# pratyushkumar211/industrial_nnmpc_2021

Measured on AMD Instinct MI355X. Metric: condensed-QP solves/sec (CDU offline datagen), higher is better.
Workload: dtype f64; 1 GPU; cdu_offline_data: synthetic CDU-size plant (n=4480 vars, m=8960 box rows, n_aug=284), 100000 sampled x0 per GPU per step, whole sequences u* written out; batch_per_gpu=100000, total_batch=100000, method=auto, parallelism=dp1 (sharded samples, 1 RCCL gather of the first moves pe...

## Files before the change

industrial_nnmpc_2021_amd/csrc/qp_asm.h:

```cpp
#pragma once
#include <hip/hip_runtime.h>
#include <stdint.h>
#include <type_traits>

#if defined(ASM_WG_TU) && ASM_WG_TU >= 0
#define ASM_OWN_KERNELS 0
#else
#define ASM_OWN_KERNELS 1
#endif

namespace nnmpc {

constexpr int ASM_MLDS = 176;
constexpr int ASM_TS = 16 * 17;
enum { ASM_RUN = 0, ASM_DONE = 1, ASM_FALLBACK = 2, ASM_CERT = 3, ASM_WIDE = 4, ASM_INVALID = 5 };
constexpr int ASM_NBIN = 8;
constexpr int ASM_NREG = 6;
constexpr int ASM_NCNT = 40;
constexpr int ASM_CNT_F32 = 16;
constexpr int ASM_NLIST = 2 * ASM_NBIN;
constexpr int ASM_BIG32 = 256;
constexpr int ASM_CNT_BIG64 = 37;
constexpr int ASM_CNT_BIG32 = 36;
constexpr int ASM_BIG32B = 384;
// ... 376 lines not shown
  if (tid == 0) *s_bad = 0;
  const size_t o = (size_t)p * d.np;
  const unsigned char* st = d.st + (size_t)p * d.n;
  const int mb = (m + 15) / 16;
  __syncthreads();
  for (int i = tid; i < mb * 16; i += 256) {
    double v = 0.0;
    if (i < m) {
      const int a = idx[i], k = a % d.nu;
      v = d.xunc[o + a] - (st[a] == 1 ? d.ub[(size_t)p * d.nu + k] : d.lb[(size_t)p * d.nu + k]);
    }
    rA[i] = v;
  }
  const int ntile = mb * (mb + 1) / 2;
  {
    const int ti = tid >> 4, tj = tid & 15;
    int I = 0, J = 0;
    for (int t0 = 0; t0 < ntile; t0 += 4) {
      double v[4];
      int tI[4], tJ[4];
#pragma unroll
      for (int u = 0; u < 4; ++u) {
        tI[u] = I; tJ[u] = J;
        const int gi = 16 * I + ti, gj = 16 * J + tj;
        v[u] = gi == gj ? 1.0 : 0.0;
        if (t0 + u < ntile && gi < m && gj < m) v[u] = d.H[(size_t)idx[gi] * d.np + idx[gj]];
        if (++J > I) { J = 0; ++I; }
      }
#pragma unroll
      for (int u = 0; u < 4; ++u)
        if (t0 + u < ntile) asm_tile(T, tI[u], tJ[u])[ti * 17 + tj] = v[u];
    }
  }
  __syncthreads();
  for (int K = 0; K < mb; ++K) {
    double* TKK = asm_tile(T, K, K);
    if (wave == 0) {
      const int bad = asm_diag16_call(TKK, Yt, lane);
      if (bad && lane == 0) *s_bad = 1;
    }
    __syncthreads();
    for (int I = K + 1 + wave; I < mb; I += 4) {
      double* TIK = asm_tile(T, I, K);
      const f64x4_t acc = tile_mma_nt(TIK, Yt, lane);
#pragma unroll
      for (int r = 0; r < 4; ++r) TIK[((lane >> 4) + 4 * r) * 17 + (lane & 15)] = acc[r];
    }
    __syncthreads();
    {
      int b = 0;
      for (int I = K + 1; I < mb; ++I)
        for (int J = K + 1; J <= I; ++J, ++b) {
          if ((b & 3) != wave) continue;
          const f64x4_t acc = tile_mma_nt(asm_tile(T, I, K), asm_tile(T, J, K), lane);
          double* TIJ = asm_tile(T, I, J);
#pragma unroll
          for (int r = 0; r < 4; ++r) TIJ[((lane >> 4) + 4 * r) * 17 + (lane & 15)] -= acc[r];
        }
    }
    if (wave == 0 && lane < 16) {
      const int row = lane;
#pragma unroll
      for (int k = 0; k < 16; ++k) if (k >= row) TKK[row * 17 + k] = Yt[k * 17 + row];
    }
    __syncthreads();
  }
  if (*s_bad) return 1;
  if (wave == 0) {
    const int i = lane & 15, kq = lane >> 4;
    for (int K = 0; K < mb; ++K) {
      double t = 0.0;
      for (int J = 0; J < K; ++J) {
        const double* TKJ = asm_tile(T, K, J);
#pragma unroll
        for (int k = 0; k < 4; ++k) t += TKJ[i * 17 + 4 * kq + k] * rA[16 * J + 4 * kq + k];
      }
      t += __shfl_xor(t, 16); t += __shfl_xor(t, 32);
      t = rA[16 * K + i] - t;
      const double* TKK = asm_tile(T, K, K);
      double yv = t * TKK[i * 17 + i];
#pragma unroll
      for (int k = 0; k < 16; ++k) { const double tk = __shfl(t, k); if (k < i) yv += TKK[k * 17 + i] * tk; }
      if (lane < 16) rA[16 * K + i] = yv;
      asm volatile("s_waitcnt lgkmcnt(0)" ::: "memory");
    }
    for (int K = mb - 1; K >= 0; --K) {
      double t = 0.0;
      for (int I = K + 1; I < mb; ++I) {
        const double* TIK = asm_tile(T, I, K);
#pragma unroll
        for (int k = 0; k < 4; ++k) t += TIK[(4 * kq + k) * 17 + i] * rA[16 * I + 4 * kq + k];
      }
      t += __shfl_xor(t, 16); t += __shfl_xor(t, 32);
      t = rA[16 * K + i] - t;
      const double* TKK = asm_tile(T, K, K);
      double lv = t * TKK[i * 17 + i];
#pragma unroll
      for (int k = 0; k < 16; ++k) { const double tk = __shfl(t, k); if (k > i) lv += TKK[i * 17 + k] * tk; }
      if (lane < 16) rA[16 * K + i] = lv;
      asm volatile("s_waitcnt lgkmcnt(0)" ::: "memory");
    }
  }
  __syncthreads();
  return 0;
}

#if ASM_OWN_KERNELS
template <int BIG>
__global__ __launch_bounds__(256, 4) void asm_lambda_tile_k(AsmDev d, int bin) {
  extern __shared__ __attribute__((aligned(16))) double sm[];
  __shared__ int s_bad;
  const int tid = threadIdx.x;
  const int cap = BIG ? d.max_active : asm_bin_cap(bin);
  double* rA = sm;
  double* Yt = rA + cap;
  double* T = BIG ? d.scratch + (size_t)blockIdx.x * ((size_t)(cap / 16) * (cap / 16 + 1) / 2 * ASM_TS)
                  : Yt + ASM_TS;
  const int nitem = BIG ? d.counters[1] : d.counters[4 + bin];
  const int* list = BIG ? d.biglist : d.binlist + (size_t)bin * d.nseg;
  for (int it = blockIdx.x; it < nitem; it += gridDim.x) {
    const int p = list[it];
    const int* idx = d.idxg + (size_t)p * d.max_active;
    const int m = d.mg[p];
    if (asm_tile_solve(d, p, m, idx, rA, Yt, T, &s_bad)) { if (tid == 0) d.state[p] = ASM_FALLBACK; continue; }
    if (tid == 0) d.prec[p] = 1;
    double* lrow = d.lam + (size_t)d.row[p] * d.np;
    for (int i = tid; i < m; i += 256) lrow[idx[i]] = rA[i];
  }
}
#endif

template <class T> struct AsmNum;
typedef float f32x4_t __attribute__((ext_vector_type(4)));
template <> struct AsmNum<double> {
  using v4 = f64x4_t;
  static constexpr bool F32 = false;
  __host__ __device__ static constexpr int kr(int lq, int r) { return lq + 4 * r; }
  __device__ static __forceinline__ v4 mfma(double a, double b, v4 c) { return __builtin_amdgcn_mfma_f64_16x16x4f64(a, b, c, 0, 0, 0); }
  __device__ static __forceinline__ double rdlane(double x, int l) { return rdlane_d(x, l); }
  __device__ static __forceinline__ double rsq(double x) { return rsqrt(x); }

  template <int CTRL> __device__ static __forceinline__ double dpp(double x) {
    const int lo = __builtin_amdgcn_mov_dpp(__double2loint(x), CTRL, 0xf, 0xf, false);
    const int hi = __builtin_amdgcn_mov_dpp(__double2hiint(x), CTRL, 0xf, 0xf, false);
    return __hiloint2double(hi, lo);
  }
  __device__ static __forceinline__ double swap16(double x) {
    const auto a = __builtin_amdgcn_permlane16_swap(__double2loint(x), __double2loint(x), false, false);
    const auto b = __builtin_amdgcn_permlane16_swap(__double2hiint(x), __double2hiint(x), false, false);
    return __hiloint2double(b[0], a[0]) + __hiloint2double(b[1], a[1]);
  }
  __device__ static __forceinline__ double swap32(double x) {
    const auto a = __builtin_amdgcn_permlane32_swap(__double2loint(x), __double2loint(x), false, false);
    const auto b = __builtin_amdgcn_permlane32_swap(__double2hiint(x), __double2hiint(x), false, false);
    return __hiloint2double(b[0], a[0]) + __hiloint2double(b[1], a[1]);
  }
};
template <> struct AsmNum<float> {
  using v4 = f32x4_t;
  static constexpr bool F32 = true;
  __host__ __device__ static constexpr int kr(int lq, int r) { return 4 * lq + r; }
  __device__ static __forceinline__ v4 mfma(float a, float b, v4 c) { return __builtin_amdgcn_mfma_f32_16x16x4f32(a, b, c, 0, 0, 0); }
  __device__ static __forceinline__ float rdlane(float x, int l) { return __int_as_float(__builtin_amdgcn_readlane(__float_as_int(x), l)); }
  __device__ static __forceinline__ float rsq(float x) { return __builtin_amdgcn_rsqf(x); }

  template <int CTRL> __device__ static __forceinline__ float dpp(float x) {
    return __int_as_float(__builtin_amdgcn_mov_dpp(__float_as_int(x), CTRL, 0xf, 0xf, false));
  }
  __device__ static __forceinline__ float swap16(float x) {
    const auto a = __builtin_amdgcn_permlane16_swap(__float_as_int(x), __float_as_int(x), false, false);
    return __int_as_float(a[0]) + __int_as_float(a[1]);
  }
  __device__ static __forceinline__ float swap32(float x) {
    const auto a = __builtin_amdgcn_permlane32_swap(__float_as_int(x), __float_as_int(x), false, false);
    return __int_as_float(a[0]) + __int_as_float(a[1]);
  }
};
template <class T> __device__ __forceinline__ T rowsum16(T x) {
  using N = AsmNum<T>;
  x += N::template dpp<0xB1>(x);
  x += N::template dpp<0x4E>(x);
  x += N::template dpp<0x141>(x);
  x += N::template dpp<0x140>(x);
  return x;
}
template <class T> __device__ __forceinline__ void rowsum16x4(T (&v)[4]) {
#pragma unroll
  for (int r = 0; r < 4; ++r) v[r] = rowsum16<T>(v[r]);
}
template <> __device__ __forceinline__ void rowsum16x4<float>(float (&v)[4]) {
  asm volatile(
      "s_nop 1\n"
      "v_add_f32_dpp %0, %0, %0 quad_perm:[1,0,3,2] row_mask:0xf bank_mask:0xf\n"
      "v_add_f32_dpp %1, %1, %1 quad_perm:[1,0,3,2] row_mask:0xf bank_mask:0xf\n"
      "v_add_f32_dpp %2, %2, %2 quad_perm:[1,0,3,2] row_mask:0xf bank_mask:0xf\n"
      "v_add_f32_dpp %3, %3, %3 quad_perm:[1,0,3,2] row_mask:0xf bank_mask:0xf\n"
      "v_add_f32_dpp %0, %0, %0 quad_perm:[2,3,0,1] row_mask:0xf bank_mask:0xf\n"
      "v_add_f32_dpp %1, %1, %1 quad_perm:[2,3,0,1] row_mask:0xf bank_mask:0xf\n"
      "v_add_f32_dpp %2, %2, %2 quad_perm:[2,3,0,1] row_mask:0xf bank_mask:0xf\n"
      "v_add_f32_dpp %3, %3, %3 quad_perm:[2,3,0,1] row_mask:0xf bank_mask:0xf\n"
      "v_add_f32_dpp %0, %0, %0 row_half_mirror row_mask:0xf bank_mask:0xf\n"
      "v_add_f32_dpp %1, %1, %1 row_half_mirror row_mask:0xf bank_mask:0xf\n"
      "v_add_f32_dpp %2, %2, %2 row_half_mirror row_mask:0xf bank_mask:0xf\n"
      "v_add_f32_dpp %3, %3, %3 row_half_mirror row_mask:0xf bank_mask:0xf\n"
      "v_add_f32_dpp %0, %0, %0 row_mirror row_mask:0xf bank_mask:0xf\n"
      "v_add_f32_dpp %1, %1, %1 row_mirror row_mask:0xf bank_mask:0xf\n"
      "v_add_f32_dpp %2, %2, %2 row_mirror row_mask:0xf bank_mask:0xf\n"
      "v_add_f32_dpp %3, %3, %3 row_mirror row_mask:0xf bank_mask:0xf\n"
      "s_nop 1\n"
      : "+v"(v[0]), "+v"(v[1]), "+v"(v[2]), "+v"(v[3]));
}
template <class T> __device__ __forceinline__ T xsum4(T x) { return AsmNum<T>::swap32(AsmNum<T>::swap16(x)); }

#ifndef ASM_NL_OF_8
#define ASM_NL_OF_8 2
#endif
template <class T> __host__ __device__ constexpr int asm_nl(int mb) {
  return mb <= 7 ? 0 : (mb == 8 ? ASM_NL_OF_8 : (mb <= 9 ? 2 : 4));
}
template <class T> __host__ __device__ constexpr int asm_nlt(int mb) { return asm_nl<T>(mb) * (mb - 1) - asm_nl<T>(mb) * (asm_nl<T>(mb) - 1) / 2; }
template <class T> __host__ __device__ constexpr int asm_rw(int mb) { return 2 * ASM_TS + 2 * mb * 16 + asm_nlt<T>(mb) * 256; }

__host__ __device__ constexpr int asm_tix(int I, int J) { return I * (I + 1) / 2 + J; }
__host__ __device__ constexpr int asm_tri_row(int n, int t) { int J = 0; while (t >= n - J) { t -= n - J; ++J; } return J; }
__host__ __device__ constexpr int asm_tri_col(int n, int t) { int J = 0; while (t >= n - J) { t -= n - J; ++J; } return J + t; }
template <int V> struct asm_ic { static constexpr int value = V; };
template <int B, int E, class F>
__device__ __forceinline__ void asm_sfor(F&& f) {
  if constexpr (B < E) { f(asm_ic<B>{}); asm_sfor<B + 1, E>(f); }
}

template <class T> __device__ __forceinline__ void asm_diag16_begin(T (&x)[16], const T* Tk, const T* Id, int lane) {
  const T* src = lane >= 32 ? Id : Tk;
  const int row = lane & 15;
#pragma unroll
  for (int k = 0; k < 16; ++k) x[k] = src[row * 17 + k];
}
template <class T, int CC> __device__ __forceinline__ void asm_diag16_step(T (&x)[16]) {
  using N = AsmNum<T>;
  const T dd = N::rdlane(x[CC], CC);
  const T w = x[CC] * N::rsq(dd);
  x[CC] = w;
#pragma unroll
  for (int c2 = CC + 1; c2 < 16; ++c2) x[c2] -= w * N::rdlane(w, c2);
}
template <class T> __device__ __forceinline__ int asm_diag16_end(const T (&x)[16], T* Yt, int lane) {
  using N = AsmNum<T>;
  const int bad = !(N::rdlane(x[15], 15) > T(0));
  if (lane >= 48) {
    const int row = lane & 15;
#pragma unroll
    for (int k = 0; k < 16; ++k) Yt[k * 17 + row] = x[k];
  }
  return bad;
}

template <class T>
__device__ __forceinline__ int asm_diag16(const T* Tk, T* Yt, int lane, const T* Id) {
  using N = AsmNum<T>;
  const int row = lane & 15;
  const bool inv_half = lane >= 32;
  T x[16];
  if (Id) {
    const T* src = inv_half ? Id : Tk;
#pragma unroll
    for (int k = 0; k < 16; ++k) x[k] = src[row * 17 + k];
  } else {
#pragma unroll
    for (int k = 0; k < 16; ++k) {
      T a = Tk[row * 17 + k];
      asm volatile("" : "+v"(a));
      x[k] = inv_half ? (k == row ? T(1) : T(0)) : a;
    }
  }
#pragma unroll
  for (int cc = 0; cc < 16; ++cc) {
    const T dd = N::rdlane(x[cc], cc);
    const T w = x[cc] * N::rsq(dd);
    x[cc] = w;
#pragma unroll
    for (int c2 = cc + 1; c2 < 16; ++c2) x[c2] -= w * N::rdlane(w, c2);
  }
  const int bad = !(N::rdlane(x[15], 15) > T(0));
  if (lane >= 48) {
#pragma unroll
    for (int k = 0; k < 16; ++k) Yt[k * 17 + row] = x[k];
  }
  return bad;
}

__device__ __noinline__ int asm_diag16_call(const double* Tk, double* Yt, int lane) { return asm_diag16<double>(Tk, Yt, lane); }


#ifdef ASM_STAMPS
__device__ unsigned long long asm_stamp_buf[64];
#ifndef ASM_STAMP_WG
#define ASM_STAMP_WG 0
#endif
#define ASM_STAMP(i) do { if (wg == ASM_STAMP_WG && wave == 0) { const unsigned long long t_ = __builtin_amdgcn_s_memtime(); if (lane == 0) asm_stamp_buf[i] = t_; } } while (0)
#else
#define ASM_STAMP(i) do { } while (0)
#endif

template <int MB> struct AsmRefine {
  const double *xunc, *lb, *ub;
  const unsigned char* st;
  const int* idx;
  double lam64[MB];
};
template <class T, int MB, int NL, bool ANYM, bool REF>
__device__ __forceinline__ int asm_reg_core(const AsmDev& d, int m, const int* ix, T* dt, T* Yt, T* ys, const T* rv, T* lt, const T* idt,
                                            T (&lam)[MB], int lane, int wg, int wave, AsmRefine<MB>& rf, bool do_refine) {
  using N = AsmNum<T>;
  using V4 = typename N::v4;
  const int li = lane & 15, lq = lane >> 4;
  auto slot = [](int I, int J) { return J * (MB - 1) - J * (J - 1) / 2 + I - J - 1; };
  (void)wg; (void)wave;
  ASM_STAMP(60);
  V4 C[MB * (MB + 1) / 2];
  {
    int gcol[MB];
#pragma unroll
    for (int I = 0; I < MB; ++I) gcol[I] = ix[16 * I + li];
    using HT0 = typename std::conditional<N::F32, float, double>::type;
    const char* const Hbase = N::F32 ? reinterpret_cast<const char*>(d.H32) : reinterpret_cast<const char*>(d.H);
    unsigned gco[MB];
#pragma unroll
    for (int I = 0; I < MB; ++I) gco[I] = (unsigned)gcol[I] * (unsigned)sizeof(HT0);
#pragma unroll
    for (int J = 0; J < MB; ++J) {
#pragma unroll
      for (int r = 0; r < 4; ++r) {
        const int gj = 16 * J + N::kr(lq, r);
        using HT = typename std::conditional<N::F32, float, double>::type;
        const unsigned rowoff = (unsigned)ix[gj] * (unsigned)d.np * (unsigned)sizeof(HT);
#pragma unroll
        for (int I = J; I < MB; ++I) {
          const int gi = 16 * I + li;
          const HT v = *reinterpret_cast<const HT*>(Hbase + (rowoff + gco[I]));
          const bool edge = ANYM || MB <= 4 || I == MB - 1;
          const T e = !edge ? (T)(-v) : ((gi < m && gj < m) ? (T)(-v) : (gi == gj ? T(-1) : T(0)));
          if (J < NL && I > J) lt[slot(I, J) * 256 + r * 64] = e;
          else C[asm_tix(I, J)][r] = e;
        }
      }
      __builtin_amdgcn_sched_barrier(0);
    }
  }
  ASM_STAMP(1);
  T ps[MB];
#pragma unroll
  for (int I = 0; I < MB; ++I) ps[I] = T(0);
  int bad = 0;
  auto trail = [&](auto Kc, auto Jc, auto Ic, const V4* P) {
    constexpr int K = decltype(Kc)::value, J = decltype(Jc)::value, I = decltype(Ic)::value;
    constexpr bool in_lds = J < NL && I > J;
    V4 acc;
    if (in_lds) {
#pragma unroll
      for (int r = 0; r < 4; ++r) acc[r] = lt[slot(I, J) * 256 + r * 64];
    } else {
      acc = C[asm_tix(I, J)];
    }
    const V4 a = K < NL ? P[J] : C[asm_tix(J, K)], b = K < NL ? P[I] : C[asm_tix(I, K)];
#pragma unroll
    for (int s4 = 0; s4 < 4; ++s4) acc = N::mfma(a[s4], b[s4], acc);
    if (in_lds) {
#pragma unroll
      for (int r = 0; r < 4; ++r) lt[slot(I, J) * 256 + r * 64] = acc[r];
    } else {
      C[asm_tix(I, J)] = acc;
    }
  };
#pragma unroll
  for (int r = 0; r < 4; ++r) dt[li * 17 + N::kr(lq, r)] = -C[asm_tix(0, 0)][r];
  ASM_FENCE();
  ASM_STAMP(2);
  bad |= asm_diag16<T>(dt, Yt, lane, idt);
  ASM_FENCE();
  ASM_STAMP(3);
  asm_sfor<0, MB>([&](auto Kc) {
    constexpr int K = decltype(Kc)::value;
    __builtin_amdgcn_sched_barrier(0);
    ASM_STAMP(4 + 3 * K);
    T yf[4];
    V4 Yc;
#pragma unroll
    for (int s4 = 0; s4 < 4; ++s4) { yf[s4] = -Yt[li * 17 + N::kr(lq, s4)]; Yc[s4] = Yt[N::kr(lq, s4) * 17 + li]; }
    C[asm_tix(K, K)] = Yc;
    const T tK = rv[16 * K + li] - (K ? xsum4<T>(ps[K]) : T(0));
    T yq[4];
#pragma unroll
    for (int r = 0; r < 4; ++r) yq[r] = Yc[r] * tK;
    rowsum16x4<T>(yq);
    if (li == 0) {
#pragma unroll
      for (int r = 0; r < 4; ++r) ys[16 * K + N::kr(lq, r)] = yq[r];
    }
    V4 P[MB];
#pragma unroll
    for (int I = K + 1; I < MB; ++I) {
      V4 b;
      if (K < NL) {
#pragma unroll
        for (int r = 0; r < 4; ++r) b[r] = lt[slot(I, K) * 256 + r * 64];
      } else {
        b = C[asm_tix(I, K)];
      }
      V4 acc = {T(0), T(0), T(0), T(0)};
#pragma unroll
      for (int s4 = 0; s4 < 4; ++s4) acc = N::mfma(yf[s4], b[s4], acc);
      if (K < NL) {
        P[I] = acc;
#pragma unroll
        for (int r = 0; r < 4; ++r) lt[slot(I, K) * 256 + r * 64] = acc[r];
      } else {
        C[asm_tix(I, K)] = acc;
      }
#pragma unroll
      for (int r = 0; r < 4; ++r) ps[I] += acc[r] * yq[r];
    }
    ASM_STAMP(5 + 3 * K);
    if constexpr (K + 1 < MB) {
      trail(Kc, asm_ic<K + 1>{}, asm_ic<K + 1>{}, P);
#pragma unroll
      for (int r = 0; r < 4; ++r) dt[li * 17 + N::kr(lq, r)] = -C[asm_tix(K + 1, K + 1)][r];
      ASM_FENCE();
      __builtin_amdgcn_sched_barrier(0);
#ifdef ASM_REG_ILV
      {
        constexpr int NR = (MB - K - 1) * (MB - K) / 2 - 1;
        T x[16];
        asm_diag16_begin<T>(x, dt, idt, lane);
        asm_sfor<0, 16>([&](auto cc) __attribute__((always_inline)) {
          constexpr int c = decltype(cc)::value;
          asm_diag16_step<T, c>(x);
          asm_sfor<c * NR / 16, (c + 1) * NR / 16>([&](auto tc) __attribute__((always_inline)) {
            constexpr int t = decltype(tc)::value + 1;
            constexpr int J = asm_tri_row(MB - K - 1, t), I = asm_tri_col(MB - K - 1, t);
            trail(Kc, asm_ic<K + 1 + J>{}, asm_ic<K + 1 + I>{}, P);
          });
          __builtin_amdgcn_sched_barrier(0);
        });
        ASM_STAMP(6 + 3 * K);
        bad |= asm_diag16_end<T>(x, Yt, lane);
        ASM_FENCE();
      }
#else
      asm_sfor<K + 1, MB>([&](auto Jc) {
        constexpr int J = decltype(Jc)::value;
        asm_sfor<J, MB>([&](auto Ic) {
          constexpr int I = decltype(Ic)::value;
          if constexpr (!(I == K + 1 && J == K + 1)) trail(Kc, Jc, Ic, P);
        });
      });
      ASM_STAMP(6 + 3 * K);
      bad |= asm_diag16<T>(dt, Yt, lane, idt);
      ASM_FENCE();
#endif
    }
  });
  ASM_STAMP(40);
  if (bad) return 1;
  ASM_FENCE();
  auto backward = [&](T (&out)[MB]) __attribute__((always_inline)) {
#pragma unroll
    for (int K = MB - 1; K >= 0; --K) {
      T part = T(0);
      T s4[4] = {T(0), T(0), T(0), T(0)};
      if (K < MB - 1) {
#pragma unroll
        for (int r = 0; r < 4; ++r)
#pragma unroll
          for (int I = K + 1; I < MB; ++I) s4[r] += (K < NL ? lt[slot(I, K) * 256 + r * 64] : C[asm_tix(I, K)][r]) * out[I];
        rowsum16x4<T>(s4);
      }
#pragma unroll
      for (int r = 0; r < 4; ++r) part += C[asm_tix(K, K)][r] * (ys[16 * K + N::kr(lq, r)] - s4[r]);
      out[K] = xsum4<T>(part);
      __builtin_amdgcn_sched_barrier(0);
    }
  };
  backward(lam);
  if constexpr (REF) {
    if (!do_refine) return 0;
    int ai[MB], sa[MB];
    double bb[MB], bnd[MB];
    bool wrong = false;
#pragma unroll
    for (int I = 0; I < MB; ++I) ai[I] = rf.idx[min(16 * I + li, m - 1)];
#pragma unroll
    for (int I = 0; I < MB; ++I) { sa[I] = rf.st[ai[I]]; bb[I] = rf.xunc[ai[I]]; }
#pragma unroll
    for (int I = 0; I < MB; ++I) { const int k = ai[I] % d.nu; bnd[I] = sa[I] == 1 ? rf.ub[k] : rf.lb[k]; }
#pragma unroll
    for (int I = 0; I < MB; ++I) {
      const bool in = 16 * I + li < m;
      bb[I] = in ? bb[I] - bnd[I] : 0.0;
      const double l = (double)lam[I];
      wrong |= in && ((sa[I] == 1 && l <= 0.0) || (sa[I] == 2 && l >= 0.0));
    }
#ifndef ASM_REFINE_ALWAYS
    if (__any(wrong)) return 0;
#endif
    int* ixr = reinterpret_cast<int*>(const_cast<T*>(rv));
    double* l64 = reinterpret_cast<double*>(dt);
    static_assert(16 * MB * 8 <= 2 * ASM_TS * (int)sizeof(T) || !N::F32, "lam64 does not fit the diagonal-tile buffers");
    unsigned gco[MB];
#pragma unroll
    for (int I = 0; I < MB; ++I) {
      gco[I] = (unsigned)ai[I] * 8u;
      if (lq == 0) { ixr[16 * I + li] = ai[I]; l64[16 * I + li] = 16 * I + li < m ? (double)lam[I] : 0.0; }
    }
    ASM_FENCE();
    const char* const H64 = reinterpret_cast<const char*>(d.H);
    double acc[MB];
#pragma unroll
    for (int I = 0; I < MB; ++I) acc[I] = 0.0;
    {
      double hv[2][MB], lj[2];
      auto issue = [&](int jj, auto bc) __attribute__((always_inline)) {
        constexpr int b = decltype(bc)::value;
        const int j = 4 * jj + lq;
        const unsigned rowoff = (unsigned)ixr[j] * (unsigned)d.np * 8u;
        lj[b] = l64[j];
#pragma unroll
        for (int I = 0; I < MB; ++I) hv[b][I] = *reinterpret_cast<const double*>(H64 + (rowoff + gco[I]));
      };
      issue(0, asm_ic<0>{});
#pragma unroll 1
      for (int jj = 0; jj < 4 * MB; jj += 2) {
        __builtin_amdgcn_sched_barrier(0);
        issue(jj + 1, asm_ic<1>{});
        __builtin_amdgcn_sched_barrier(0);
#pragma unroll
        for (int I = 0; I < MB; ++I) acc[I] = fma(hv[0][I], lj[0], acc[I]);
        __builtin_amdgcn_sched_barrier(0);
        issue(min(jj + 2, 4 * MB - 1), asm_ic<0>{});
        __builtin_amdgcn_sched_barrier(0);
#pragma unroll
        for (int I = 0; I < MB; ++I) acc[I] = fma(hv[1][I], lj[1], acc[I]);
      }
    }
    T rr[MB];
#pragma unroll
    for (int I = 0; I < MB; ++I) rr[I] = 16 * I + li < m ? (T)(bb[I] - xsum4<double>(acc[I])) : T(0);
#pragma unroll
    for (int I = 0; I < MB; ++I) ps[I] = T(0);
    asm_sfor<0, MB>([&](auto Kc) __attribute__((always_inline)) {
      constexpr int K = decltype(Kc)::value;
      const V4 Yc = C[asm_tix(K, K)];
      const T tK = rr[K] - (K ? xsum4<T>(ps[K]) : T(0));
      T yq[4];
#pragma unroll
      for (int r = 0; r < 4; ++r) yq[r] = Yc[r] * tK;
      rowsum16x4<T>(yq);
      if (li == 0) {
#pragma unroll
        for (int r = 0; r < 4; ++r) ys[16 * K + N::kr(lq, r)] = yq[r];
      }
#pragma unroll
      for (int I = K + 1; I < MB; ++I)
#pragma unroll
        for (int r = 0; r < 4; ++r) ps[I] += (K < NL ? lt[slot(I, K) * 256 + r * 64] : C[asm_tix(I, K)][r]) * yq[r];
      __builtin_amdgcn_sched_barrier(0);
    });
    ASM_FENCE();
    T dl[MB];
    backward(dl);
#pragma unroll
    for (int I = 0; I < MB; ++I) rf.lam64[I] = (double)lam[I] + (double)dl[I];
    return 2;
  }
  return 0;
}
template <class T, int MB, int NL = asm_nl<T>(MB), bool ANYM = false>
__device__ __forceinline__ int asm_reg_core(const AsmDev& d, int m, const int* ix, T* dt, T* Yt, T* ys, const T* rv, T* lt, const T* idt,
                                            T (&lam)[MB], int lane, int wg, int wave) {
  AsmRefine<MB> none;
  return asm_reg_core<T, MB, NL, ANYM, false>(d, m, ix, dt, Yt, ys, rv, lt, idt, lam, lane, wg, wave, none, false);
}

template <class T, int MB, int WPB>
__device__ __forceinline__ void asm_lambda_reg(const AsmDev& d, int list, int wg) {
  using N = AsmNum<T>;
  extern __shared__ __attribute__((aligned(16))) unsigned char sm_raw[];
  const int tid = threadIdx.x, lane = tid & 63, wave = __builtin_amdgcn_readfirstlane(tid >> 6);
  const int li = lane & 15, lq = lane >> 4;
  T* dt = reinterpret_cast<T*>(sm_raw) + (size_t)wave * asm_rw<T>(MB);
  T* Yt = dt + ASM_TS;
  T* ys = Yt + ASM_TS;
  T* rv = ys + MB * 16;
  T* lt = rv + MB * 16 + lane;
  T* idt = reinterpret_cast<T*>(sm_raw) + (size_t)WPB * asm_rw<T>(MB);
  for (int i = lane; i < ASM_TS; i += 64) idt[i] = (i / 17 == i % 17) ? T(1) : T(0);
  const int nitem = d.counters[asm_list_counter(list)];
  const int it = wg * WPB + wave;
  if (it >= nitem) return;
  const int p = __builtin_amdgcn_readfirstlane(d.binlist[(size_t)list * d.nseg + it]);
  const size_t o = (size_t)p * d.np;
  const unsigned char* st = d.st + (size_t)p * d.n;
  const int* idx = d.idxg + (size_t)p * d.max_active;
  const int m = __builtin_amdgcn_readfirstlane(d.mg[p]);
  if (m <= 0) return;
  ASM_STAMP(0);
  int* ix = reinterpret_cast<int*>(ys);
  for (int i = lane; i < MB * 16; i += 64) {
    const int a = idx[min(i, m - 1)], k = a % d.nu;
    ix[i] = a;
    const double v = d.xunc[o + a] - (st[a] == 1 ? d.ub[(size_t)p * d.nu + k] : d.lb[(size_t)p * d.nu + k]);
    rv[i] = i < m ? (T)v : T(0);
  }
  ASM_FENCE();
  T lam[MB];
  AsmRefine<MB> rf;
  const bool refine = N::F32 && d.rowk[p] == 0;
  if (N::F32) { rf.xunc = d.xunc + o; rf.lb = d.lb + (size_t)p * d.nu; rf.ub = d.ub + (size_t)p * d.nu; rf.st = st; rf.idx = idx; }
  const int bad = asm_reg_core<T, MB, asm_nl<T>(MB), false, N::F32>(d, m, ix, dt, Yt, ys, rv, lt, idt, lam, lane, wg, wave, rf, refine);
  if (N::F32 && refine && bad != 1) {
    if (bad == 2 && lane == 0) d.redo[p] = 2;
    double* lrow64 = d.lam + (size_t)d.row[p] * d.np;
#pragma unroll
    for (int I = 0; I < MB; ++I) {
      const int i = 16 * I + li;
      if (lq == 0 && i < m) lrow64[idx[i]] = bad == 2 ? rf.lam64[I] : (double)lam[I];
    }
    return;
  }
  if (bad) {
    if (lane == 0) { if (N::F32) { d.prec[p] = 1; d.redo[p] = 1; } else d.state[p] = ASM_FALLBACK; }
    return;
  }
  if (!N::F32 && lane == 0) d.prec[p] = 1;
  ASM_STAMP(41);
  using LT = typename std::conditional<N::F32, float, double>::type;
  LT* lrow = (N::F32 ? (LT*)d.lam32 : (LT*)d.lam) + (size_t)d.row[p] * d.np;
#pragma unroll
  for (int I = 0; I < MB; ++I) {
    const int i = 16 * I + li;
    if (lq == 0 && i < m) lrow[idx[i]] = (LT)lam[I];
  }
}

typedef float f32x4v_t __attribute__((ext_vector_type(4)));
__device__ __forceinline__ f32x4v_t tile_mma_nt32(const float* A, const float* B, int lane) {
  f32x4v_t acc = {0.f, 0.f, 0.f, 0.f};
  const int li = lane & 15, kq = lane >> 4;
#pragma unroll
  for (int s = 0; s < 4; ++s)
    acc = __builtin_amdgcn_mfma_f32_16x16x4f32(A[li * 17 + 4 * s + kq], B[li * 17 + 4 * s + kq], acc, 0, 0, 0);
  return acc;
}
__device__ __forceinline__ float* asm_tile32(float* T, int I, int J) { return T + ((size_t)I * (I + 1) / 2 + J) * ASM_TS; }

__device__ __forceinline__ int asm_tile_solve32(const AsmDev& d, int p, int m, const int* idx, float* rA, float* Yt, float* T, int* s_bad) {
  const int tid = threadIdx.x, lane = tid & 63, wave = tid >> 6;
#ifdef ASM_STAMPS
  const int wg = blockIdx.x;
#endif
  __syncthreads();
  ASM_STAMP(48);
  if (tid == 0) *s_bad = 0;
  const size_t o = (size_t)p * d.np;
  const unsigned char* st = d.st + (size_t)p * d.n;
  const int mb = (m + 15) / 16;
  __syncthreads();
  for (int i = tid; i < mb * 16; i += 512) {
    float v = 0.f;
    if (i < m) {
      const int a = idx[i], k = a % d.nu;
      v = (float)(d.xunc[o + a] - (st[a] == 1 ? d.ub[(size_t)p * d.nu + k] : d.lb[(size_t)p * d.nu + k]));
    }
    rA[i] = v;
  }
  const int ntile = mb * (mb + 1) / 2;
  {
    const int half = tid >> 8, ti = (tid >> 4) & 15, tj = tid & 15;
    for (int t0 = half; t0 < ntile; t0 += 2 * 8) {
      float v[8];
      int tt[8];
#pragma unroll
      for (int u = 0; u < 8; ++u) {
        const int t = t0 + 2 * u;
        int I = (int)((sqrtf(8.f * (float)t + 1.f) - 1.f) * 0.5f);
        while ((I + 1) * (I + 2) / 2 <= t) ++I;
        while (I * (I + 1) / 2 > t) --I;
        const int J = t - I * (I + 1) / 2;
        tt[u] = t;
        const int gi = 16 * I + ti, gj = 16 * J + tj;
        v[u] = gi == gj ? 1.f : 0.f;
        if (t < ntile && gi < m && gj < m) v[u] = d.H32[(size_t)idx[gi] * d.np + idx[gj]];
      }
#pragma unroll
      for (int u = 0; u < 8; ++u)
        if (tt[u] < ntile) (T + (size_t)tt[u] * ASM_TS)[ti * 17 + tj] = v[u];
    }
  }
  __syncthreads();
  ASM_STAMP(49);
  if (wave == 0) {
    const int bad = asm_diag16<float>(asm_tile32(T, 0, 0), Yt, lane);
    if (bad && lane == 0) *s_bad = 1;
  }
  __syncthreads();
  ASM_STAMP(50);
  for (int K = 0; K < mb; ++K) {
    float* TKK = asm_tile32(T, K, K);
    for (int I = K + 1 + wave; I < mb; I += 8) {
      float* TIK = asm_tile32(T, I, K);
      const f32x4v_t acc = tile_mma_nt32(TIK, Yt, lane);
#pragma unroll
      for (int r = 0; r < 4; ++r) TIK[(4 * (lane >> 4) + r) * 17 + (lane & 15)] = acc[r];
    }
    __syncthreads();
    if (wave == 0) {
      if (lane < 16) {
        const int row = lane;
#pragma unroll
        for (int k = 0; k < 16; ++k) if (k >= row) TKK[row * 17 + k] = Yt[k * 17 + row];
      }
      if (K + 1 < mb) {
        const f32x4v_t acc = tile_mma_nt32(asm_tile32(T, K + 1, K), asm_tile32(T, K + 1, K), lane);
        float* Tn = asm_tile32(T, K + 1, K + 1);
#pragma unroll
        for (int r = 0; r < 4; ++r) Tn[(4 * (lane >> 4) + r) * 17 + (lane & 15)] -= acc[r];
        asm volatile("s_waitcnt lgkmcnt(0)" ::: "memory");
        const int bad = asm_diag16<float>(Tn, Yt, lane);
        if (bad && lane == 0) *s_bad = 1;
      }
    } else {
      int b = 0;
      for (int I = K + 1; I < mb; ++I)
        for (int J = K + 1; J <= I; ++J) {
          if (I == K + 1) continue;
          if ((b++ % 7) + 1 != wave) continue;
          const f32x4v_t acc = tile_mma_nt32(asm_tile32(T, I, K), asm_tile32(T, J, K), lane);
          float* TIJ = asm_tile32(T, I, J);
#pragma unroll
          for (int r = 0; r < 4; ++r) TIJ[(4 * (lane >> 4) + r) * 17 + (lane & 15)] -= acc[r];
        }
    }
    __syncthreads();
  }
  ASM_STAMP(51);
  if (*s_bad) return 1;
  {
    const int i = lane & 15, kq = lane >> 4;
    for (int K = 0; K < mb; ++K) {
      if (wave == 0) {
        const float* TKK = asm_tile32(T, K, K);
        const float t = rA[16 * K + i];
        float yv = t * TKK[i * 17 + i];
#pragma unroll
        for (int k = 0; k < 16; ++k) { const float tk = __shfl(t, k); if (k < i) yv += TKK[k * 17 + i] * tk; }
        asm volatile("s_waitcnt lgkmcnt(0)" ::: "memory");
        if (lane < 16) rA[16 * K + i] = yv;
      }
      __syncthreads();
      for (int I = K + 1 + wave; I < mb; I += 8) {
        const float* TIK = asm_tile32(T, I, K);
        float t = 0.f;
#pragma unroll
        for (int k = 0; k < 4; ++k) t += TIK[i * 17 + 4 * kq + k] * rA[16 * K + 4 * kq + k];
        t += __shfl_xor(t, 16); t += __shfl_xor(t, 32);
        if (lane < 16) rA[16 * I + i] -= t;
      }
      __syncthreads();
    }
    for (int K = mb - 1; K >= 0; --K) {
      if (wave == 0) {
        const float* TKK = asm_tile32(T, K, K);
        const float t = rA[16 * K + i];
        float lv = t * TKK[i * 17 + i];
#pragma unroll
        for (int k = 0; k < 16; ++k) { const float tk = __shfl(t, k); if (k > i) lv += TKK[i * 17 + k] * tk; }
        asm volatile("s_waitcnt lgkmcnt(0)" ::: "memory");
        if (lane < 16) rA[16 * K + i] = lv;
      }
      __syncthreads();
      for (int J = K - 1 - wave; J >= 0; J -= 8) {
        const float* TKJ = asm_tile32(T, K, J);
        float t = 0.f;
#pragma unroll
        for (int k = 0; k < 4; ++k) t += TKJ[(4 * kq + k) * 17 + i] * rA[16 * K + 4 * kq + k];
        t += __shfl_xor(t, 16); t += __shfl_xor(t, 32);
        if (lane < 16) rA[16 * J + i] -= t;
      }
      __syncthreads();
    }
  }
  ASM_STAMP(52);
  __syncthreads();
  return 0;
}

constexpr int ASM_TILE32_LDS = (ASM_BIG32 + ASM_TS + (ASM_BIG32 / 16) * (ASM_BIG32 / 16 + 1) / 2 * ASM_TS) * 4;
#if ASM_OWN_KERNELS
__global__ __launch_bounds__(512, 1) void asm_lambda_tile32_k(AsmDev d) {
  extern __shared__ __attribute__((aligned(16))) float smf[];
  __shared__ int s_bad;
  const int tid = threadIdx.x;
  float* rA = smf;
  float* Yt = rA + ASM_BIG32;
  float* T = Yt + ASM_TS;
  const int nitem = d.counters[ASM_CNT_BIG32];
  const int* list = d.binlist + (size_t)ASM_NLIST * d.nseg;
  for (int it = blockIdx.x; it < nitem; it += gridDim.x) {
    const int p = list[it];
    const int* idx = d.idxg + (size_t)p * d.max_active;
    const int m = d.mg[p];
    if (asm_tile_solve32(d, p, m, idx, rA, Yt, T, &s_bad)) {
      if (tid == 0) { d.prec[p] = 1; d.redo[p] = 1; }
      continue;
    }
    float* lrow = d.lam32 + (size_t)d.row[p] * d.np;
    for (int i = tid; i < m; i += 512) lrow[idx[i]] = rA[i];
  }
}
#endif

constexpr int ASM_REG_LDS = (4 * asm_rw<double>(ASM_NREG + 3) + ASM_TS) * 8;
#if ASM_OWN_KERNELS
__global__ __launch_bounds__(256, 1) void asm_lambda_reg_k(AsmDev d) {
  int w = blockIdx.x;
#define ASM_REG_CLASS(B)                                                   \
  {                                                                        \
    const int nb = (d.counters[4 + B] + 3) >> 2;                           \
    if (w < nb) { asm_lambda_reg<double, B + 4, 4>(d, B, w); return; }     \
    w -= nb;                                                               \
  }
  ASM_REG_CLASS(5) ASM_REG_CLASS(4) ASM_REG_CLASS(3) ASM_REG_CLASS(2) ASM_REG_CLASS(1) ASM_REG_CLASS(0)
#undef ASM_REG_CLASS
  static_assert(ASM_NREG == 6, "one ASM_REG_CLASS line per register-resident size class");
}
#endif
constexpr int ASM_REG2_LDS = (2 * asm_rw<double>(11) + ASM_TS) * 8;
#if ASM_OWN_KERNELS
__global__ __launch_bounds__(128, 1) void asm_lambda_reg2_k(AsmDev d) {
  int w = blockIdx.x;
  {
    const int nb = (d.counters[4 + 7] + 1) >> 1;
    if (w < nb) { asm_lambda_reg<double, 11, 2>(d, 7, w); return; }
    w -= nb;
  }
  asm_lambda_reg<double, 10, 2>(d, 6, w);
  static_assert(ASM_NBIN == 8 && ASM_MLDS == 176, "classes 6 and 7 are the 10- and 11-block sets");
}
#endif
constexpr int ASM_REG32_LDS = (4 * asm_rw<float>(ASM_NREG + 3) + ASM_TS) * 4;
#if ASM_OWN_KERNELS
__global__ __launch_bounds__(256, 2) void asm_lambda_reg32_k(AsmDev d) {
  int w = blockIdx.x;
#define ASM_REG_CLASS(B)                                                            \
  {                                                                                 \
    const int nb = (d.counters[ASM_CNT_F32 + B] + 3) >> 2;                          \
    if (w < nb) { asm_lambda_reg<float, B + 4, 4>(d, ASM_NBIN + B, w); return; }    \
    w -= nb;                                                                        \
  }
  ASM_REG_CLASS(5) ASM_REG_CLASS(4) ASM_REG_CLASS(3) ASM_REG_CLASS(2) ASM_REG_CLASS(1) ASM_REG_CLASS(0)
#undef ASM_REG_CLASS
}
#endif

constexpr int ASM_REG32B_LDS = (4 * asm_rw<float>(11) + ASM_TS) * 4;
#if ASM_OWN_KERNELS
__global__ __launch_bounds__(256, 1) void asm_lambda_reg32b_k(AsmDev d) {
  int w = blockIdx.x;
// ... 810 lines not shown
```

Measured before the change: 7.422 million solves/s.

## Exploit Hessian symmetry in refinement residual for small active-set blocks

For active-set block counts up to a configurable limit, the refinement residual H*lambda now reads only the lower-triangular blocks of H. Each loaded entry is used twice: once for the row product and once, via a row reduction written to LDS, for the transposed contribution. This is meant to roughly halve global loads of H during refinement, at the cost of extra reductions, LDS traffic and register pressure. The backward-solve and forward-solve loops are also rewritten with compile-time index loops and if-constexpr so that dead branches are removed at compile time.

```diff
diff --git a/industrial_nnmpc_2021_amd/csrc/qp_asm.h b/industrial_nnmpc_2021_amd/csrc/qp_asm.h
--- a/industrial_nnmpc_2021_amd/csrc/qp_asm.h
+++ b/industrial_nnmpc_2021_amd/csrc/qp_asm.h
@@ -702,6 +702,9 @@
 #define ASM_STAMP(i) do { } while (0)
 #endif
 
+#ifndef ASM_REFINE_LOWER_MAXMB
+#define ASM_REFINE_LOWER_MAXMB 4
+#endif
 template <int MB> struct AsmRefine {
   const double *xunc, *lb, *ub;
   const unsigned char* st;
@@ -864,22 +867,25 @@
   if (bad) return 1;
   ASM_FENCE();
   auto backward = [&](T (&out)[MB]) __attribute__((always_inline)) {
-#pragma unroll
-    for (int K = MB - 1; K >= 0; --K) {
+    asm_sfor<0, MB>([&](auto Rc) __attribute__((always_inline)) {
+      constexpr int K = MB - 1 - decltype(Rc)::value;
       T part = T(0);
       T s4[4] = {T(0), T(0), T(0), T(0)};
-      if (K < MB - 1) {
+      if constexpr (K < MB - 1) {
 #pragma unroll
         for (int r = 0; r < 4; ++r)
-#pragma unroll
-          for (int I = K + 1; I < MB; ++I) s4[r] += (K < NL ? lt[slot(I, K) * 256 + r * 64] : C[asm_tix(I, K)][r]) * out[I];
+          asm_sfor<K + 1, MB>([&](auto Ic) __attribute__((always_inline)) {
+            constexpr int I = decltype(Ic)::value;
+            if constexpr (K < NL) s4[r] += lt[slot(I, K) * 256 + r * 64] * out[I];
+            else s4[r] += C[asm_tix(I, K)][r] * out[I];
+          });
         rowsum16x4<T>(s4);
       }
 #pragma unroll
       for (int r = 0; r < 4; ++r) part += C[asm_tix(K, K)][r] * (ys[16 * K + N::kr(lq, r)] - s4[r]);
       out[K] = xsum4<T>(part);
       __builtin_amdgcn_sched_barrier(0);
-    }
+    });
   };
   backward(lam);
   if constexpr (REF) {
@@ -903,9 +909,11 @@
 #ifndef ASM_REFINE_ALWAYS
     if (__any(wrong)) return 0;
 #endif
-    int* ixr = reinterpret_cast<int*>(const_cast<T*>(rv));
     double* l64 = reinterpret_cast<double*>(dt);
     static_assert(16 * MB * 8 <= 2 * ASM_TS * (int)sizeof(T) || !N::F32, "lam64 does not fit the diagonal-tile buffers");
+    constexpr bool LOWER = MB <= ASM_REFINE_LOWER_MAXMB;
+    int* ixr = LOWER ? reinterpret_cast<int*>(l64 + 16 * MB) : reinterpret_cast<int*>(const_cast<T*>(rv));
+    static_assert(!LOWER || 16 * MB * 12 <= 2 * ASM_TS * (int)sizeof(T) || !N::F32, "lam64 and the index list do not fit the diagonal-tile buffers");
     unsigned gco[MB];
 #pragma unroll
     for (int I = 0; I < MB; ++I) {
@@ -917,7 +925,8 @@
     double acc[MB];
 #pragma unroll
     for (int I = 0; I < MB; ++I) acc[I] = 0.0;
-    {
+    T rr[MB];
+    if constexpr (!LOWER) {
       double hv[2][MB], lj[2];
       auto issue = [&](int jj, auto bc) __attribute__((always_inline)) {
         constexpr int b = decltype(bc)::value;
@@ -941,10 +950,65 @@
 #pragma unroll
         for (int I = 0; I < MB; ++I) acc[I] = fma(hv[1][I], lj[1], acc[I]);
       }
-    }
-    T rr[MB];
-#pragma unroll
-    for (int I = 0; I < MB; ++I) rr[I] = 16 * I + li < m ? (T)(bb[I] - xsum4<double>(acc[I])) : T(0);
+#pragma unroll
+      for (int I = 0; I < MB; ++I) rr[I] = 16 * I + li < m ? (T)(bb[I] - xsum4<double>(acc[I])) : T(0);
+    } else {
+      double* tt = reinterpret_cast<double*>(ys);
+      double hv[2][MB];
+      auto issue = [&](int J, auto sc, auto bc) __attribute__((always_inline)) {
+        constexpr int b = decltype(bc)::value;
+        const int j = 16 * J + 4 * decltype(sc)::value + lq;
+        const unsigned rowoff = (unsigned)ixr[j] * (unsigned)d.np * 8u;
+        asm_sfor<0, MB>([&](auto Ic) __attribute__((always_inline)) {
+          constexpr int I = decltype(Ic)::value;
+          hv[b][I] = *reinterpret_cast<const double*>(H64 + (I >= J ? rowoff + gco[I] : 0u));
+        });
+      };
+      auto use = [&](int J, auto sc, auto bc) __attribute__((always_inline)) {
+        constexpr int b = decltype(bc)::value;
+        const int j = 16 * J + 4 * decltype(sc)::value + lq;
+        const double lj = l64[j];
+        double tp = 0.0;
+        asm_sfor<0, MB>([&](auto Ic) __attribute__((always_inline)) {
+          constexpr int I = decltype(Ic)::value;
+          if (I >= J) {
+            acc[I] = fma(hv[b][I], lj, acc[I]);
+            if (I > J) {
+              T lf = lam[I];
+              asm volatile("" : "+v"(lf));
+              const double lid = (MB <= 4 || I == MB - 1) && !(16 * I + li < m) ? 0.0 : (double)lf;
+              tp = fma(hv[b][I], lid, tp);
+            }
+          }
+        });
+        tp = rowsum16<double>(tp);
+        if (li == 0) tt[j] = tp;
+      };
+      issue(0, asm_ic<0>{}, asm_ic<0>{});
+#pragma unroll 1
+      for (int J = 0; J < MB; ++J) {
+        __builtin_amdgcn_sched_barrier(0);
+        issue(J, asm_ic<1>{}, asm_ic<1>{});
+        __builtin_amdgcn_sched_barrier(0);
+        use(J, asm_ic<0>{}, asm_ic<0>{});
+        __builtin_amdgcn_sched_barrier(0);
+        issue(J, asm_ic<2>{}, asm_ic<0>{});
+        __builtin_amdgcn_sched_barrier(0);
+        use(J, asm_ic<1>{}, asm_ic<1>{});
+        __builtin_amdgcn_sched_barrier(0);
+        issue(J, asm_ic<3>{}, asm_ic<1>{});
+        __builtin_amdgcn_sched_barrier(0);
+        use(J, asm_ic<2>{}, asm_ic<0>{});
+        __builtin_amdgcn_sched_barrier(0);
+        issue(min(J + 1, MB - 1), asm_ic<0>{}, asm_ic<0>{});
+        __builtin_amdgcn_sched_barrier(0);
+        use(J, asm_ic<3>{}, asm_ic<1>{});
+      }
+      ASM_FENCE();
+#pragma unroll
+      for (int I = 0; I < MB; ++I) rr[I] = 16 * I + li < m ? (T)(bb[I] - (xsum4<double>(acc[I]) + tt[16 * I + li])) : T(0);
+      ASM_FENCE();
+    }
 #pragma unroll
     for (int I = 0; I < MB; ++I) ps[I] = T(0);
     asm_sfor<0, MB>([&](auto Kc) __attribute__((always_inline)) {
@@ -959,10 +1023,14 @@
 #pragma unroll
         for (int r = 0; r < 4; ++r) ys[16 * K + N::kr(lq, r)] = yq[r];
       }
-#pragma unroll
-      for (int I = K + 1; I < MB; ++I)
-#pragma unroll
-        for (int r = 0; r < 4; ++r) ps[I] += (K < NL ? lt[slot(I, K) * 256 + r * 64] : C[asm_tix(I, K)][r]) * yq[r];
+      asm_sfor<K + 1, MB>([&](auto Ic) __attribute__((always_inline)) {
+        constexpr int I = decltype(Ic)::value;
+#pragma unroll
+        for (int r = 0; r < 4; ++r) {
+          if constexpr (K < NL) ps[I] += lt[slot(I, K) * 256 + r * 64] * yq[r];
+          else ps[I] += C[asm_tix(I, K)][r] * yq[r];
+        }
+      });
       __builtin_amdgcn_sched_barrier(0);
     });
     ASM_FENCE();
```

New measurement: 7.526 million solves/s, median of 6. 1.01x the previous value.
